# google/balloon-learning-environment

Measured on AMD Instinct MI355X. Metric: env-steps/sec at 65 536 parallel envs; achieved HBM GB/s fraction of peak, higher is better.
Workload: dtype f32+f64

## Files before the change

balloon_learning_environment_amd/csrc/ble_physics.h:

```cpp
#pragma once
#include "ble_intrinsics.h"

#ifndef BLE_STEP_EVENT
#define BLE_STEP_EVENT(i) do {} while (0)
#endif
#ifndef BLE_STEP_TICK
#define BLE_STEP_TICK(i) do {} while (0)
#endif

namespace ble {

constexpr float kGravity = 9.80665f;
constexpr double kGasConstantD = 8.3144621;
constexpr double kAirMolarMassD = 0.028964922481160;
constexpr double kHeMolarMassD = 0.004002602;
constexpr double kAirSpecificGasD = kGasConstantD / kAirMolarMassD;
constexpr float kAirMolarOverR = (float)(kAirMolarMassD / kGasConstantD);
constexpr float kGasConstant = (float)kGasConstantD;
constexpr double kPiD = 3.14159265358979323846;
constexpr float kPi = (float)kPiD;
constexpr float kDegToRad = (float)(kPiD / 180.0);
constexpr float kRadToDeg = (float)(180.0 / kPiD);

constexpr float kVolumeBase = 1804.0f;
// ... 75 lines not shown
  return d_fma(d_fma(-q0, b, x), rb, q0);
}
BLE_FN double d_rcp(double x) {
  double r = d_rcp_seed(x);
  return d_fma(d_fma(-x, r, 1.0), r, r);
}
BLE_FN double d_rsqrt(double x) {
  double y = d_rsq_seed(x);
  return y * d_fma(-0.5 * x * y, y, 1.5);
}
BLE_FN double d_sqrt_rs(double x) { return x * d_rsqrt(x); }
BLE_FN double d_sqrt_fast(double x) {
  double y = d_rsqrt(x);
  double sq = x * y;
  return d_fma(0.5 * y, d_fma(-sq, sq, x), sq);
}
constexpr double kThermalMu = 1.458e-6 / (0.028964922481160 / 8.3144621);
constexpr double kRayleighScale = 9.80665 * (1.0 / kThermalMu) * (1.0 / kThermalMu) * (6.0 / 3.14159265358979323846);
constexpr double kRayleighT = -3.25e-4 * kRayleighScale, kRayleighT0 = 0.804 * kRayleighScale;
constexpr double kEmitRho = 1.0 / (1.0 - 0.0291), kEmitC1 = 0.000232, kEmitC0 = 0.04587 - 0.000232 * 210.0;
constexpr double kEmitA = 0.000000056704 * (-kEmitRho * kEmitC1 * kEmitC1);
constexpr double kEmitB = 0.000000056704 * (2.0 * kEmitC1 - 2.0 * kEmitRho * kEmitC1 * kEmitC0);
constexpr double kEmitC = 0.000000056704 * (2.0 * kEmitC0 - kEmitRho * kEmitC0 * kEmitC0);
constexpr double kCondTenth = 0.1 * (0.0241 * 0.006415624181362592) / (2.0 * 0.62035049089940009);
struct StrideK {
  double ra_t0, five, eleven, emit_b, emit_c;
  double dry_mass;
  double lg5, lg4, lg3, ex4, ex3;
  double acs_x0, forty;
  double t110, cond_tenth;
  double m_over_r, ten;
  double lg6, ex5;
  double lift, v0;
};
BLE_FN StrideK stride_k_literal(double dry_mass = VehicleDefault::dry_mass, double lift = VehicleDefault::lift, double v0 = VehicleDefault::v0) {
  StrideK k;
  k.ra_t0 = kRayleighT0; k.five = 5.0; k.eleven = 11.0; k.emit_b = kEmitB; k.emit_c = kEmitC;
  k.dry_mass = dry_mass;
  k.lg5 = 0.2; k.lg4 = -0.25; k.lg3 = 1.0 / 3.0; k.ex4 = 1.0 / 24.0; k.ex3 = 1.0 / 6.0;
  k.acs_x0 = 0.05; k.forty = 40.0;
  k.t110 = 110.4; k.cond_tenth = kCondTenth;
  k.m_over_r = kAirMolarMassD / kGasConstantD; k.ten = 10.0;
  k.lg6 = -1.0 / 6.0; k.ex5 = 1.0 / 120.0;
  k.lift = lift; k.v0 = v0;
  return k;
}
BLE_FN StrideK stride_k_vreg(double dry_mass = VehicleDefault::dry_mass, double lift = VehicleDefault::lift, double v0 = VehicleDefault::v0) {
  StrideK k = stride_k_literal(dry_mass, lift, v0);
  k.ra_t0 = d_vreg(k.ra_t0); k.five = d_vreg(k.five); k.eleven = d_vreg(k.eleven); k.emit_b = d_vreg(k.emit_b); k.emit_c = d_vreg(k.emit_c);
  k.dry_mass = d_vreg(k.dry_mass);
  k.lg5 = d_vreg(k.lg5); k.lg4 = d_vreg(k.lg4); k.lg3 = d_vreg(k.lg3); k.ex4 = d_vreg(k.ex4); k.ex3 = d_vreg(k.ex3);
  k.acs_x0 = d_vreg(k.acs_x0); k.forty = d_vreg(k.forty);
  k.t110 = d_vreg(k.t110); k.cond_tenth = d_vreg(k.cond_tenth);
  k.m_over_r = d_vreg(k.m_over_r); k.ten = d_vreg(k.ten);
  k.lg6 = d_vreg(k.lg6); k.ex5 = d_vreg(k.ex5);
  k.lift = d_vreg(k.lift); k.v0 = d_vreg(k.v0);
  return k;
}
BLE_FN double d_log_fast(double x) {
  double m = d_frexp_mant(x);
  int e = d_frexp_exp(x);
  if (m < 0.70710678118654752) { m *= 2.0; e -= 1; }
  double sq = (m - 1.0) * d_rcp(m + 1.0);
  double z = sq * sq;
  double pl = 1.0 / 23.0;
  pl = d_fma(pl, z, 1.0 / 21.0); pl = d_fma(pl, z, 1.0 / 19.0); pl = d_fma(pl, z, 1.0 / 17.0);
  pl = d_fma(pl, z, 1.0 / 15.0); pl = d_fma(pl, z, 1.0 / 13.0); pl = d_fma(pl, z, 1.0 / 11.0);
  pl = d_fma(pl, z, 1.0 / 9.0); pl = d_fma(pl, z, 1.0 / 7.0); pl = d_fma(pl, z, 0.2);
  pl = d_fma(pl, z, 1.0 / 3.0);
  double lm = d_fma(2.0 * sq * z, pl, 2.0 * sq);
  double de = (double)e;
  return d_fma(de, 6.93147180369123816490e-01, d_fma(de, 1.90821492927058770002e-10, lm));
}
BLE_FN double d_exp_fast(double t) {
  double kq = d_rint(t * 1.44269504088896338700e+00);
  double r = d_fma(kq, -6.93147180369123816490e-01, t);
  r = d_fma(kq, -1.90821492927058770002e-10, r);
  double pe = 1.0 / 6227020800.0;
  pe = d_fma(pe, r, 1.0 / 479001600.0); pe = d_fma(pe, r, 1.0 / 39916800.0); pe = d_fma(pe, r, 1.0 / 3628800.0);
  pe = d_fma(pe, r, 1.0 / 362880.0); pe = d_fma(pe, r, 1.0 / 40320.0); pe = d_fma(pe, r, 1.0 / 5040.0);
  pe = d_fma(pe, r, 1.0 / 720.0); pe = d_fma(pe, r, 1.0 / 120.0); pe = d_fma(pe, r, 1.0 / 24.0);
  pe = d_fma(pe, r, 1.0 / 6.0); pe = d_fma(pe, r, 0.5); pe = d_fma(pe, r, 1.0); pe = d_fma(pe, r, 1.0);
  return d_ldexp(pe, (int)kq);
}
BLE_FN double d_pow_fast(double x, double y) { return d_exp_fast(y * d_log_fast(x)); }

constexpr float kLog2e = 1.4426950408889634f;
constexpr float kLn2 = 0.6931471805599453f;
BLE_FN float f_exp(float x) { return f_exp2(x * kLog2e); }
// ... 271 lines not shown
  double r = c0;
  r = j < 0 ? m1 : r;
  r = j > 0 ? p1 : r;
  return r;
}
BLE_FN double atm_height_rel_boundary_f64(double q, double pb, double r_pb, double tb, double lapse) {
  const double x = (q - pb) * r_pb;
  const double lg = x * d_fma(x, d_fma(x, d_fma(x, -0.25, 1.0 / 3.0), -0.5), 1.0);
  if (lapse == 0.0) return (-kAirSpecificGasD / 9.80665) * tb * lg;
  const double y = (-kAirSpecificGasD / 9.80665) * lapse * lg;
  const double em1 = y * d_fma(y, d_fma(y, d_fma(y, 1.0 / 24.0, 1.0 / 6.0), 0.5), 1.0);
  return (tb * em1) * d_rcp(lapse);
}
BLE_FN double atm_inv_delta_height_f64(const AtmWindow& w, int j, double lapse, double kl, double cur_hi, double cur_lo,
                                       double p, double rp, double d, double t_p, const StrideK& K = stride_k_literal()) {
  const double x = d * rp;
  const double lg = x * d_fma(x, d_fma(x, K.lg3, -0.5), 1.0);
  const bool iso = lapse == 0.0;
  const double y = kl * lg;
  const double em1 = y * d_fma(y, d_fma(y, K.ex3, 0.5), 1.0);
  double inv = lapse * d_rcp(t_p * em1);
  if (__builtin_expect(wave_any(iso), 0)) if (iso) inv = d_rcp(t_p * ((-kAirSpecificGasD / 9.80665) * lg));
  const double q = p + d;
  const bool below = q > cur_hi;
  const bool above = !(q > cur_lo);
  if (__builtin_expect(wave_any(below || above), 0)) if (below || above) {
    BLE_STEP_EVENT(2);
    const bool at_pb = (j == 0) ? below : (j < 0);
    const double pb = at_pb ? w.pb : w.pt, r_pb = at_pb ? w.r_pb : w.r_pt, tb = at_pb ? w.tb : w.tt;
    const double lapse_q = pick3(below ? j - 1 : j + 1, w.lapse_m1, w.lapse_0, w.lapse_p1);
    const double dh = atm_height_rel_boundary_f64(q, pb, r_pb, tb, lapse_q) -
                      atm_height_rel_boundary_f64(p, pb, r_pb, tb, lapse);
    inv = d_rcp(dh);
  }
  return inv;
}

BLE_FN int atm_window_layer(const AtmWindow& w, double p) { return p > w.pb ? -1 : (p > w.pt ? 0 : 1); }
BLE_FN AtmLayer atm_layer_f32(const AtmWindow& w, int j) {
  const float inf = __builtin_huge_valf();
  AtmLayer l;
  const float pb = (float)w.pb, pt = (float)w.pt, tb = (float)w.tb, tt = (float)w.tt;
  l.p_base = j < 0 ? inf : (j == 0 ? pb : pt);
  l.t_base = j == 0 ? tb : tt;
  l.p_top = j < 0 ? pb : (j == 0 ? pt : -inf);
  l.t_top = j < 0 ? tb : tt;
  const float lm1 = (float)w.lapse_m1, l0 = (float)w.lapse_0, lp1 = (float)w.lapse_p1;
  l.lapse = j < 0 ? lm1 : (j == 0 ? l0 : lp1);
  l.lapse_below = j <= 0 ? lm1 : l0;
  l.lapse_above = j < 0 ? l0 : lp1;
  l.h_base = (float)w.hb; l.k = -kROverG * l.lapse; l.index = w.i0 + j;
  return l;
}

BLE_FN int altitude_safety(int action, double altitude_m, uint8_t* fsm) {
  const double min_alt = 50000.0 * 0.3048, buffer = 500.0 * 0.3048, hyst = 500.0 * 0.3048;
  int s = *fsm;
  if (altitude_m < min_alt) s = 2;
  else if (altitude_m < min_alt + buffer) s = 1;
  else if (altitude_m < min_alt + buffer + hyst) s = (s == 2 || s == 1) ? 1 : 0;
  else s = 0;
  *fsm = (uint8_t)s;
  if (s == 2) return kUp;
  if (s == 1 && action == kDown) return kStay;
  return action;
}
// ... 450 lines not shown
  return f_fma(c35x4, sh33, c65x2 * sh27);
}
BLE_FN float solar_power_from_factor(float panel_factor, float attenuation) { return 210.0f * attenuation * panel_factor; }
BLE_FN float solar_power(const SunState& sun, float attenuation) {
  return solar_power_from_factor(solar_panel_factor(sun), attenuation);
}

constexpr float kSolarAbsorptivityTotal =
    0.01435f * (1.0f + (1.0f - 0.01435f - 0.0291f) / (1.0f - 0.0291f));
BLE_FN double d_inv_root4(double a, double five = 5.0) {
  const double y = (double)f_sqrt(f_rsqrt((float)a));
  const double y2 = y * y;
  return y * d_fma(-a * y2, y2, five) * 0.25;
}
BLE_FN double d_inv_root10(double a, double eleven = 11.0, double scale = 0.1) {
  const double y = (double)f_exp2(-0.1f * f_log2((float)a));
  const double y2 = y * y, y4 = y2 * y2, y5 = y4 * y;
  return y * d_fma(-a * y5, y5, eleven) * scale;
}
constexpr double kStefanBoltzmannD = 0.000000056704;
BLE_FN double total_absorptivity_d(double a) { return a * d_fma(-a, 1.0 / (1.0 - 0.0291), 2.0); }
constexpr double kAbsTLo = 0x1.891a7b9611a78p+3;
constexpr double kAbsTHi = 0x1.05f0e58469ee5p+13;
BLE_FN bool absorptivity_out_of_range(double t_k) { return t_k < kAbsTLo || t_k > kAbsTHi; }
constexpr float kAbsIrLo = 0x1.52847cp-10f;
constexpr float kAbsIrHi = 0x1.0af2d6p+28f;
BLE_FN bool earth_ir_out_of_range(double ir) { return ir < (double)kAbsIrLo || ir > (double)kAbsIrHi; }
BLE_FN double earth_heat_per_area_f64(double upwelling_ir, uint32_t* flags) {
  const double t_bb = d_sqrt(d_sqrt(upwelling_ir * (1.0 / kStefanBoltzmannD)));
  const double f = total_absorptivity_d(d_fma(0.000232, t_bb - 210.0, 0.04587));
  *flags |= earth_ir_out_of_range(upwelling_ir) ? kFlagAbsorptivity : 0u;
  return upwelling_ir * 0.4605 * f;
}
template <bool kExactTwelfthRoot = false>
BLE_FN double thermal_increment_f64(double vol, double yc, double t_int, double t_amb, double p, double q_solar_area,
                                    double q_earth_area, const StrideK& K = stride_k_literal(), double thermal_scale = VehicleDefault::thermal_scale) {
  constexpr double kR2 = 0.38483473658887897;
  constexpr double kR1 = 0.62035049089940009;
  const double v23 = vol * yc;
  const double t2 = t_int * t_int;
  const double q_emit = (t2 * t2) * d_fma(d_fma(kEmitA, t_int, K.emit_b), t_int, K.emit_c);
  const double rt = d_rcp(t_amb), rt2 = rt * rt, rt3 = rt2 * rt;
  const double pw = p * (t_amb + K.t110);
  const double dt = t_amb - t_int;
  double ra = (d_fma(kRayleighT, t_amb, K.ra_t0) * (pw * pw)) * ((vol * (rt3 * rt3)) * __builtin_fabs(dt));
  ra = d_max(ra, 1e-30);
  const double y4 = d_inv_root4(ra, K.five);
  const double ra14 = (ra * y4) * (y4 * y4);
  const double tw_arg = d_fma(2.69e-8, ra, 1.0);
  double tw = (double)f_pow((float)tw_arg, 1.0f / 12.0f);
  if (kExactTwelfthRoot) {
    const double y2 = tw * tw, y4r = y2 * y2, y8 = y4r * y4r;
    tw = d_fma(-tw * (1.0 / 12.0), d_fma(y8 * y4r, d_rcp(tw_arg), -1.0), tw);
  }
  const double nusselt = d_fma(0.457, ra14, 2.0 + tw);
  const double q_conv = ((nusselt * (t_amb * d_inv_root10(t_amb, K.eleven, K.cond_tenth))) * yc) * dt;
  const double q = (q_solar_area + q_earth_area) + (q_conv - q_emit);
  return (q * v23) * thermal_scale;
}

BLE_FN void superpressure_volume(float mols_air, float t_int, float p, float* volume, float* sp) {
  float vu = (kMolsLiftGas + mols_air) * kGasConstant * t_int * f_rcp(p);
  if (vu <= kVolumeBase) { *volume = vu; *sp = 0.0f; return; }
  float b = -(kVolumeBase - kVolumeDvDp * p);
  float c4 = 4.0f * kVolumeDvDp * vu * p;
  float v = 0.5f * (f_sqrt(f_fma(b, b, c4)) - b);
  *volume = v;
  *sp = p * (vu - v) * f_rcp(v);
}

BLE_FN void superpressure_volume_f64(double mols_air, double t_int, double p, double rp, double* volume, double* sp,
                                     const StrideK& K = stride_k_literal(), double dvdp = VehicleDefault::dvdp,
                                     double four_dvdp = VehicleDefault::four_dvdp, double inv_dvdp = VehicleDefault::inv_dvdp) {
  const double w = ((K.lift + mols_air) * kGasConstantD) * t_int;
  double vu = w * rp;
  double b = -(K.v0 - dvdp * p);
  double c4 = four_dvdp * w;
  double v = 0.5 * (d_sqrt_rs(d_fma(b, b, c4)) - b);
  bool slack = vu <= K.v0;
  *volume = slack ? vu : v;
  *sp = slack ? 0.0 : (v - K.v0) * inv_dvdp;
}

struct AcsEfficiencyTable { float v[4 * 13]; };
constexpr AcsEfficiencyTable kAcsEfficiencyValues = {{
    0.4f, 0.4f, 0.3f, 0.2f, 0.2f, 0.0f, 0.0f, 0.0f, 0.0f, 0.0f, 0.0f, 0.0f, 0.0f,
    0.4f, 0.3f, 0.3f, 0.30f, 0.25f, 0.23f, 0.20f, 0.15f, 0.12f, 0.10f, 0.0f, 0.0f, 0.0f,
    0.0f, 0.3f, 0.25f, 0.25f, 0.25f, 0.20f, 0.20f, 0.20f, 0.2f, 0.15f, 0.13f, 0.12f, 0.11f,
    0.0f, 0.23f, 0.23f, 0.23f, 0.23f, 0.23f, 0.20f, 0.20f, 0.20f, 0.18f, 0.16f, 0.15f, 0.13f}};
BLE_CONST_TABLE AcsEfficiencyTable kAcsEfficiencyTable = kAcsEfficiencyValues;
#define kAcsEfficiency (kAcsEfficiencyTable.v)
// ... 88 lines not shown
```

balloon_learning_environment_amd/csrc/ble_step_core.h:

```cpp
#pragma once
#include "ble_physics.h"

namespace ble {

struct StateDev {
  float *x, *y, *pressure, *ambient_temperature, *internal_temperature, *envelope_volume, *superpressure, *mols_air, *battery_charge;
  float *acs_power, *acs_mass_flow, *solar_charging, *power_load;
  const float *center_lat_deg, *center_lng_deg, *upwelling_infrared, *alpha;
  const int64_t* start_unix;
  int32_t *time_elapsed_s, *sunrise_h_rel, *sunset_rel;
  uint8_t *status, *last_command, *alt_fsm, *env_fsm, *power_paused;
  double* episode_cache;
};
struct EnvRegs {
  float x, y, p, t_amb, t_int, vol, sp, n_air, batt;
  float acs_power, mdot, charge, load;
  int32_t t_elapsed, sunrise_h, sunset;
  uint8_t status, alt_fsm, env_fsm, paused;
};
struct EnvConst {
  float lat0_deg, lng0_deg, ir, alpha;
  int64_t start_unix;
};
struct EnvHoisted {
// ... 40 lines not shown
}
BLE_FN EnvHoisted hoisted_from_cache(const EpisodeCacheRow& r, const EnvConst& c) {
  EnvHoisted h;
  atm_base_linear((double)c.alpha, &h.atm);
  h.atm.p1 = r.v[0]; h.atm.p2 = r.v[1];
  h.sin_lat0 = r.v[2]; h.cos_lat0 = r.v[3]; h.q_earth = r.v[4];
  uint64_t g2;
  __builtin_memcpy(&g2, &r.v[6], 8);
  h.flags = (uint32_t)(g2 & 0x7fffffffull);
  return h;
}


BLE_FN double inv_cbrt_volume(double vol) {
  double yc = (double)f_exp2((-1.0f / 3.0f) * f_log2((float)vol));
  return yc * d_fma(-vol * yc, yc * yc, 4.0) * (1.0 / 3.0);
}
BLE_FN double d_min_raw(double a, double b) {
#if defined(__HIP_DEVICE_COMPILE__)
  double r; asm("v_min_f64 %0, %1, %2" : "=v"(r) : "v"(a), "v"(b)); return r;
#else
  return d_min(a, b);
#endif
}
BLE_FN double d_max_raw(double a, double b) {
#if defined(__HIP_DEVICE_COMPILE__)
  double r; asm("v_max_f64 %0, %1, %2" : "=v"(r) : "v"(a), "v"(b)); return r;
#else
  return d_max(a, b);
#endif
}
struct LayerCursor {
  int lay;
  double lapse_cur;
  double kl_cur;
  double cur_hi, cur_lo;
};
BLE_FN double stride_pressure(const AtmWindow& win, const LayerCursor& lc, double p, double rp, double vol, double n_air,
                              double t_amb, double t_at_p, double yc, const StrideK& K, double drag_arg = VehicleDefault::drag_arg) {
  const double mass = d_fma(kAirMolarMassD, n_air, K.dry_mass);
  const double num = d_fma(p * vol, K.m_over_r, -mass * t_amb);
  const double dir = __builtin_copysign(1.0, num);
  const double arg = drag_arg * __builtin_fabs(num) * rp * (yc * yc);
  const double dh_dt = d_sqrt_rs(d_max(arg, 1e-30));
  const double inv_dh = atm_inv_delta_height_f64(win, lc.lay, lc.lapse_cur, lc.kl_cur, lc.cur_hi, lc.cur_lo, p, rp, dir, t_at_p, K);
  return d_fma(inv_dh * dh_dt, K.ten, p);
}
BLE_FN double stride_internal_temperature(double vol, double yc, double t_int, double t_amb, double p, float flux, float att,
                                          double q_earth, const StrideK& K, double thermal_scale = VehicleDefault::thermal_scale) {
  return t_int + thermal_increment_f64(vol, yc, t_int, t_amb, p, (double)((flux * att) * (0.25f * kSolarAbsorptivityTotal)), q_earth, K, thermal_scale);
}
BLE_FN void stride_acs(const double* acs_poly, int eff, double sp, double p, double rp, double t_int, float* acs_w, double* mdot_d,
                       const StrideK& K, double valve_k = VehicleDefault::valve_k) {
  const double a2 = d_max((2.0 * (kAirMolarMassD / kGasConstantD)) * (sp * (sp + p)), 1e-30);
  const double mdot_up = (valve_k * a2) * d_rsqrt(a2 * t_int);
  const double prm1 = d_max(sp * rp, 0.0);
  double w_down, mdot_down;
  acs_down_poly(acs_poly, prm1, &w_down, &mdot_down, K);
  *acs_w = eff == kDown ? (float)w_down : 0.0f;
  *mdot_d = eff == kUp ? mdot_up : (eff == kDown ? mdot_down : 0.0);
}
BLE_FN double stride_mols_air(double n_air, double mdot_d) {
  return d_max(d_fma(mdot_d, 10.0 / kAirMolarMassD, n_air), 0.0);
}
BLE_FN void stride_power_from_factor(bool is_day, float panel_factor, float att, float acs_w, float* charge, float* load, float* batt,
                                     float day_load = VehicleDefault::day_load, float night_load = VehicleDefault::night_load,
                                     float capacity = VehicleDefault::capacity) {
  *charge = is_day ? solar_power_from_factor(panel_factor, att) : 0.0f;
  *load = (is_day ? day_load : night_load) + acs_w;
  *batt = f_clamp(f_fma(*charge - *load, kStride / 3600.0f, *batt), 0.0f, capacity);
}
BLE_FN void stride_power(const SunState& sun, float att, float acs_w, float* charge, float* load, float* batt,
                         float day_load = VehicleDefault::day_load, float night_load = VehicleDefault::night_load,
                         float capacity = VehicleDefault::capacity) {
  stride_power_from_factor(sun.day, solar_panel_factor(sun), att, acs_w, charge, load, batt, day_load, night_load, capacity);
}
BLE_FN double stride_ambient_advance(const AtmWindow& win, LayerCursor& lc, double p, double rp, double t_at_p, double p_new,
                                     const StrideK& K) {
  const double kInf = (double)__builtin_huge_valf();
  double anchor_p = p, anchor_rp = rp, anchor_t = t_at_p;
  const bool crossed = p_new > lc.cur_hi || !(p_new > lc.cur_lo);
  if (__builtin_expect(wave_any(crossed), 0)) if (crossed) {
    BLE_STEP_EVENT(1);
    const int lay_new = atm_window_layer(win, p_new);
    const bool low_pair = (lc.lay + lay_new) < 0;
    anchor_p = low_pair ? win.pb : win.pt;
    anchor_rp = low_pair ? win.r_pb : win.r_pt;
    anchor_t = low_pair ? win.tb : win.tt;
    lc.lay = lay_new;
    lc.lapse_cur = pick3(lay_new, win.lapse_m1, win.lapse_0, win.lapse_p1);
    lc.kl_cur = (-kAirSpecificGasD / 9.80665) * lc.lapse_cur;
    lc.cur_hi = lay_new < 0 ? kInf : (lay_new == 0 ? win.pb : win.pt);
    lc.cur_lo = lay_new < 0 ? win.pb : (lay_new == 0 ? win.pt : -kInf);
  }
  return atm_temperature_advance(anchor_t, anchor_p, anchor_rp, p_new, lc.kl_cur, K);
}

struct SolarNodes {
  double sb0, cb0, sb1, cb1, sb2, cb2;
  double sd0, cd0, hsd, hcd;
};
BLE_FN SolarNodes solar_nodes_time(const Ephemeris& e0, int64_t t0, float lng0_deg, float step_s) {
  SolarNodes n;
  double sod;
  if (__builtin_expect(t0 >= 0 && t0 < 4294967296LL, 1)) sod = (double)((uint32_t)t0 % 86400u);
  else { int64_t m = t0 % 86400; sod = (double)(m < 0 ? m + 86400 : m); }
  const double b0 = sod * (1.0 / 240.0) + 0.25 * e0.eot_min + (double)lng0_deg;
  const double half_db = 0.5 * ((double)step_s * (1.0 / 240.0) + 0.25 * (double)(e0.eot_min_rate * step_s));
  double sb0, cb0;
  sincos_f64(b0 * (kPiD / 180.0), &sb0, &cb0);
  const double hr = half_db * (kPiD / 180.0), h2 = hr * hr;
  const double sh = hr * d_fma(h2, d_fma(h2, d_fma(h2, -1.0 / 5040.0, 1.0 / 120.0), -1.0 / 6.0), 1.0);
  const double ch = d_fma(h2, d_fma(h2, d_fma(h2, -1.0 / 720.0, 1.0 / 24.0), -0.5), 1.0);
  const double sb1 = sb0 * ch + cb0 * sh, cb1 = cb0 * ch - sb0 * sh;
  const double sb2 = sb1 * ch + cb1 * sh, cb2 = cb1 * ch - sb1 * sh;
  n.sb0 = sb0; n.cb0 = cb0; n.sb1 = sb1; n.cb1 = cb1; n.sb2 = sb2; n.cb2 = cb2;
  const double sd0 = (double)e0.sin_decl, cd0 = d_sqrt_fast(d_fma(-sd0, sd0, 1.0));
  const double hsd = 0.5 * (double)(e0.sin_decl_rate * step_s), hcd = -(sd0 * d_rcp(cd0)) * hsd;
  n.sd0 = sd0; n.cd0 = cd0; n.hsd = hsd; n.hcd = hcd;
  return n;
}
template <int j>
BLE_FN double solar_node(const SolarNodes& n, double sl0, double cl0, float x_m, float y_m, float u, float v, int substeps) {
  const double x0 = (double)x_m, y0 = (double)y_m;
  const double dx = (double)u * (5.0 * (double)substeps), dy = (double)v * (5.0 * (double)substeps);
  if (j == 0) return sun_one_minus_sin_f64(sl0, cl0, x0, y0, n.sb0, n.cb0, n.sd0, n.cd0);
// ... 44 lines not shown
    if (!excess) {
      const float scale = f_clamp((acs_power - 100.0f) * (1.0f / 200.0f), 0.0f, 1.0f);
      r *= f_fma(-0.3f, scale, 0.95f);
    }
  }
  return r;
}
template <typename SunFn>
BLE_FN float step_reward(int action, float x, float y, float p, float batt, float acs_power, SunFn sun_end,
                         float day_load = VehicleDefault::day_load, double capacity_wh = VehicleDefault::capacity_d) {
  return step_reward_from_power(action, x, y, batt, acs_power, [&]() {
    const SunState sun = sun_end();
    return solar_power(sun, solar_attenuation(sun.sin_el, p, sun.day));
  }, day_load, capacity_wh);
}

constexpr int kTermSaveRows = 14, kTermSaveStride = 64;
constexpr int kTermAbsBit = 1 << 16;
struct NoHelper { static constexpr bool kOn = false; };
struct SunRecord { float diff, panel_factor, flux; uint32_t bits; };
template <class V = VehicleDefault, class H = NoHelper>
BLE_FN int agent_step(EnvRegs& s, const EnvConst& c, const EnvHoisted& hc, int action, const WindCorners& corners, const WindQuery& wq,
                      float noise_u, float noise_v, int substeps, const double* acs_poly, const StrideK& K, float* term_save,
                      float* reward, uint32_t* flags, const V& veh = V(), H* helper = nullptr) {
  BLE_STEP_TICK(0);
  float u, v;
  if constexpr (H::kOn) {
    wind_blend_corners(corners, wq, &u, &v);
    u += noise_u; v += noise_v;
    helper->publish(s.x, s.y, u, v, s.t_elapsed);
  }
  const float p0_in = s.p;
  double p = (double)s.p;
  const AtmWindow win = atm_window_from(hc.atm, (double)c.alpha, p, flags);
  double altitude, t_at_p;
  atm_at_pressure_f64(win, (double)c.alpha, p, &altitude, &t_at_p);
  LayerCursor lc;
  lc.lay = 0; lc.lapse_cur = win.lapse_0; lc.kl_cur = (-kAirSpecificGasD / 9.80665) * win.lapse_0; lc.cur_hi = win.pb; lc.cur_lo = win.pt;

  int eff = action;
  if (veh.power_layer)
    eff = power_safety(action, s.t_elapsed, s.batt, &s.sunrise_h, &s.sunset, &s.paused, veh.night_load_d, veh.capacity_d);
  eff = envelope_safety(eff, s.sp, &s.env_fsm, veh.max_sp);
  eff = altitude_safety(eff, altitude, &s.alt_fsm);
  BLE_STEP_TICK(1);

  const int64_t t0 = c.start_unix + (int64_t)s.t_elapsed;
  const Ephemeris e0 = ephemeris(t0);
  const float step_s = (float)(10 * substeps);
  const float fl0 = e0.flux, dfl = e0.flux_rate * 10.0f;
  BLE_STEP_TICK(2);
  if constexpr (!H::kOn) {
    wind_blend_corners(corners, wq, &u, &v);
    u += noise_u; v += noise_v;
  }
  BLE_STEP_TICK(3);
  const SolarNodes nodes = solar_nodes_time(e0, t0, c.lng0_deg, step_s);
  const SunQuadratic sq = solar_nodes_site(nodes, hc.sin_lat0, hc.cos_lat0, s.x, s.y, u, v, substeps);
  BLE_STEP_TICK(4);
  const float x_start = s.x, y_start = s.y;
  const int32_t t_start = s.t_elapsed;
  auto sun_at = [&](int kk) -> SunState {
    return sun_at_stride(kk, sq, c, u, v, x_start, y_start, t_start);
  };
  const double q_earth = hc.q_earth;
  *flags |= hc.flags;

  double t_amb = (double)s.t_amb, t_int = (double)s.t_int, n_air = (double)s.n_air, vol = (double)s.vol,
         sp = (double)s.sp;
  double t_int_lo = t_int, t_int_hi = t_int;
  float x = s.x, y = s.y, batt = s.batt;
  float acs_w = s.acs_power, charge = s.charge, load = s.load;
  double mdot_d = (double)s.mdot;
  int status = kOk;

  float* const term_word = term_save + (kTermSaveRows - 1) * kTermSaveStride;
  *term_word = 0.0f;
  auto stride = [&](const int k) __attribute__((always_inline)) {
    const float pf = (float)p;
    const double rp = d_rcp(p);
    t_int_lo = d_min_raw(t_int_lo, t_int); t_int_hi = d_max_raw(t_int_hi, t_int);
    SunState sun;
    SunRecord rec;
    float flux;
    if constexpr (!H::kOn) {
      const float fk = (float)k;
      sun = sun_at(k);
      flux = f_fma(fk, dfl, fl0);
    } else {
      rec = helper->record(k);
      flux = rec.flux;
    }

    const double yc = inv_cbrt_volume(vol);
    const double p_new = stride_pressure(win, lc, p, rp, vol, n_air, t_amb, t_at_p, yc, K, veh.drag_arg);

    float att;
    if constexpr (!H::kOn) att = solar_attenuation(sun.sin_el, pf, sun.day);
    else att = solar_attenuation_from_diff(rec.diff, pf, (rec.bits & 1u) != 0);
    const double t_int_new = stride_internal_temperature(vol, yc, t_int, t_amb, p, flux, att, q_earth, K, veh.thermal_scale);

    double vol_new, sp_new;
    superpressure_volume_f64(n_air, t_int, p, rp, &vol_new, &sp_new, K, veh.dvdp, veh.four_dvdp, veh.inv_dvdp);
    bool terminal = !(sp_new <= veh.max_sp) || sp_new <= 0.0;

    stride_acs(acs_poly, eff, sp, p, rp, t_int, &acs_w, &mdot_d, K, veh.valve_k);
    const double n_air_new = stride_mols_air(n_air, mdot_d);

    if constexpr (!H::kOn) stride_power(sun, att, acs_w, &charge, &load, &batt, veh.day_load, veh.night_load, veh.capacity);
    else stride_power_from_factor((rec.bits & 1u) != 0, rec.panel_factor, att, acs_w, &charge, &load, &batt, veh.day_load, veh.night_load, veh.capacity);
    terminal = terminal || batt <= 0.0f;

    x = f_fma(u, kStride, x);
    y = f_fma(v, kStride, y);
    t_amb = t_at_p;
    t_at_p = stride_ambient_advance(win, lc, p, rp, t_at_p, p_new, K);
    p = p_new; t_int = t_int_new; vol = vol_new; sp = sp_new; n_air = n_air_new;
    if (__builtin_expect(wave_any(terminal), 0)) if (terminal && __builtin_bit_cast(int, *term_word) == 0) {
      int st = kOk;
      if (!(sp <= veh.max_sp)) st = kBurst;
      if (sp <= 0.0) st = kZeroPressure;
      if (batt <= 0.0f) st = kOutOfPower;
      const float parked[kTermSaveRows - 1] = {x, y, (float)p, (float)t_amb, (float)t_int, (float)vol, (float)sp, (float)n_air, batt,
                                               acs_w, (float)mdot_d, charge, load};
#pragma unroll
      for (int j = 0; j < kTermSaveRows - 1; ++j) term_save[j * kTermSaveStride] = parked[j];
      const int strides = i_opaque(k + 1);
      const int abs_bad = absorptivity_out_of_range(t_int_lo) || absorptivity_out_of_range(t_int_hi) ? kTermAbsBit : 0;
      *term_word = __builtin_bit_cast(float, st | (strides << 8) | abs_bad);
      if constexpr (H::kOn) helper->park_reward_record(k + 1);
    }
  };
  int ks = 0;
#pragma unroll 1
  for (; ks + 1 < substeps; ks += 2) { stride(ks); stride(ks + 1); }
  if (ks < substeps) stride(ks);
  BLE_STEP_TICK(5);
  s.x = x; s.y = y; s.p = (float)p; s.t_amb = (float)t_amb; s.t_int = (float)t_int; s.vol = (float)vol;
  s.sp = (float)sp; s.n_air = (float)n_air; s.batt = batt;
  s.acs_power = acs_w; s.mdot = (float)mdot_d; s.charge = charge; s.load = load;
  int k = substeps;
  const int word = __builtin_bit_cast(int, *term_word);
  const bool done = word != 0;
  SunRecord rec_end;
  if constexpr (H::kOn) rec_end = helper->record_end(substeps);
  bool abs_bad = absorptivity_out_of_range(t_int_lo) || absorptivity_out_of_range(t_int_hi);
  if (__builtin_expect(wave_any(done), 0)) if (done) {
    s.x = term_save[0]; s.y = term_save[kTermSaveStride]; s.p = term_save[2 * kTermSaveStride]; s.t_amb = term_save[3 * kTermSaveStride];
    s.t_int = term_save[4 * kTermSaveStride]; s.vol = term_save[5 * kTermSaveStride]; s.sp = term_save[6 * kTermSaveStride];
// ... 24 lines not shown
```

balloon_learning_environment_amd/csrc/ble_step_split.h:

```cpp
#pragma once
#include "ble_noise.h"
#include "ble_step_core.h"

#ifdef BLE_SPLIT_TIMING
#define BLE_SPLIT_T_DECL long long t_acc[6] = {0, 0, 0, 0, 0, 0}; long long t_last = (long long)__builtin_readcyclecounter()
#define BLE_SPLIT_T(sec) do { const long long t_now = (long long)__builtin_readcyclecounter(); t_acc[sec] += t_now - t_last; t_last = t_now; } while (0)
#define BLE_SPLIT_T_FLUSH(dbg, role) do { if ((dbg) != nullptr && lane == 0) { for (int q = 0; q < 6; ++q) atomicAdd((dbg) + (role) * 8 + q, (unsigned long long)t_acc[q]); atomicAdd((dbg) + (role) * 8 + 7, 1ull); } } while (0)
#else
#define BLE_SPLIT_T_DECL do {} while (0)
#define BLE_SPLIT_T(sec) do {} while (0)
#define BLE_SPLIT_T_FLUSH(dbg, role) do {} while (0)
#endif

namespace ble {

constexpr int kSplitWaves = 4;
constexpr int kSplitLanes = 64;

struct SplitShared {
  double acs_poly[kAcsPolyDoubles];
  double p[2][kSplitLanes], t_amb[2][kSplitLanes];
  float x[2][kSplitLanes], y[2][kSplitLanes];
  double t_int[2][kSplitLanes];
  float sin_el[2][kSplitLanes], panel[2][kSplitLanes]; uint32_t day[2][kSplitLanes];
// ... 77 lines not shown
      noise_draws_fetch(a.gen.seed, (uint64_t)i, (uint64_t)(i + a.gen.env_offset), a.gen.episode ? a.gen.episode[i] : 0u, a.gen.harmonic_cache, n,
                        &shn.draws[0][lane], kSplitLanes);
  }
  __syncthreads();
  const bool was_live = live;
  int last_act = 0;
  EnvHoisted hc;
  if (in_range && st.episode_cache != nullptr && episode_cache_hit(cached, c)) {
    hc = hoisted_from_cache(cached, c);
  } else {
    hc = hoist_constants(c);
    if (r0 && live && st.episode_cache != nullptr) episode_cache_store(st.episode_cache, n, i, c, hc);
  }
  int xk = 0;
  BLE_SPLIT_T_DECL;

#pragma unroll 1
  for (int step = 0; step < a.n_steps; ++step) {
    const int64_t o = (int64_t)step * n + i;
    int act = kStay;
    if (in_range) act = a.action[o];
    if (live) last_act = act;

    double p = (double)s.p, t_amb = (double)s.t_amb, t_int = (double)s.t_int, n_air = (double)s.n_air, vol = (double)s.vol,
           sp = (double)s.sp;
    float x = s.x, y = s.y, batt = s.batt;
    float acs_w = 0.0f, mdot = 0.0f, charge = 0.0f, load = 0.0f;
    float u = 0.0f, v = 0.0f;
    const float p0_in = s.p, x_start = s.x, y_start = s.y;
    const int32_t t_start = s.t_elapsed;
    const int64_t t0 = c.start_unix + (int64_t)s.t_elapsed;
    const float step_s = (float)(10 * substeps);
    uint32_t step_flags = 0;
    AtmWindow win = {}; LayerCursor lc = {}; double t_at_p = 0.0;
    float fl0 = 0.0f, dfl = 0.0f; Ephemeris e0 = {};
    SunQuadratic sq = {}; double node_f0 = 0.0;
    float sun_sin = 0.0f, sun_panel = 0.0f; bool sun_day = false;
    uint32_t map_pow_env = 0; int eff = kStay;

    if (r1) {
      e0 = ephemeris(t0);
      fl0 = e0.flux; dfl = e0.flux_rate * 10.0f;
      sh.eot_min[lane] = e0.eot_min; sh.eph[0][lane] = e0.eot_min_rate; sh.eph[1][lane] = e0.sin_decl; sh.eph[2][lane] = e0.sin_decl_rate;
      step_flags |= hc.flags;
    }
    if (r3) {
      int32_t sr0 = s.sunrise_h, ss0 = s.sunset, sr1 = s.sunrise_h, ss1 = s.sunset, sr2 = s.sunrise_h, ss2 = s.sunset;
      uint8_t pa0 = s.paused, pa1 = s.paused, pa2 = s.paused, f0 = s.env_fsm, f1 = s.env_fsm, f2 = s.env_fsm;
      const int q0 = envelope_safety(power_safety(kDown, s.t_elapsed, s.batt, &sr0, &ss0, &pa0), s.sp, &f0);
      const int q1 = envelope_safety(power_safety(kStay, s.t_elapsed, s.batt, &sr1, &ss1, &pa1), s.sp, &f1);
      const int q2 = envelope_safety(power_safety(kUp, s.t_elapsed, s.batt, &sr2, &ss2, &pa2), s.sp, &f2);
      if (live) { s.sunrise_h = sr0; s.sunset = ss0; s.paused = pa0; s.env_fsm = f0; }
      map_pow_env = action_map(q0, q1, q2);
    }
    if constexpr (kNoise) {
      if (in_range) {
        float x_km, y_km, t_h;
        noise_coords(s.x, s.y, s.t_elapsed, &x_km, &y_km, &t_h);
#pragma unroll 1
        for (int k = wave; k < 10; k += kSplitWaves)
          shn.nz[k][lane] = noise_harmonic_value(k / 5, k % 5, harmonic_draw_from_rows(&shn.draws[0][lane], kSplitLanes, k), x_km, y_km, s.p, t_h,
                                                 shn.grad_lut);
      }
      __syncthreads();
    }
    if (r2) {
      const WindQuery wq = wind_query(s.x, s.y, s.p, s.t_elapsed);
      WindCorners corners;
      wind_gather(a.wind_grid + (in_range ? i : 0) * a.grid_env_stride, wq, &corners);
      float nu = 0.0f, nv = 0.0f;
      if constexpr (kNoise) {
        if (in_range) wind_noise_from_values(&shn.nz[0][lane], kSplitLanes, &nu, &nv);
      } else {
        if (a.noise_uv && in_range) { nu = a.noise_uv[2 * i]; nv = a.noise_uv[2 * i + 1]; }
      }
      wind_blend_corners(corners, wq, &u, &v);
      u += nu; v += nv;
      sh.u[lane] = u; sh.v[lane] = v;
    }
    BLE_SPLIT_T(0);
    __syncthreads();
    BLE_SPLIT_T(1);
    if (!r2) { u = sh.u[lane]; v = sh.v[lane]; }
    if (!r1) { e0.eot_min = sh.eot_min[lane]; e0.eot_min_rate = sh.eph[0][lane]; e0.sin_decl = sh.eph[1][lane]; e0.sin_decl_rate = sh.eph[2][lane]; }
    if (r0) {
      win = atm_window_from(hc.atm, (double)c.alpha, p, &step_flags);
      lc.lay = 0; lc.lapse_cur = win.lapse_0; lc.kl_cur = (-kAirSpecificGasD / 9.80665) * win.lapse_0; lc.cur_hi = win.pb; lc.cur_lo = win.pt;
      double altitude;
      atm_at_pressure_f64(win, (double)c.alpha, p, &altitude, &t_at_p);
      uint8_t f0 = s.alt_fsm, f1 = s.alt_fsm, f2 = s.alt_fsm;
      const int q0 = altitude_safety(kDown, altitude, &f0), q1 = altitude_safety(kStay, altitude, &f1),
                q2 = altitude_safety(kUp, altitude, &f2);
      if (live) s.alt_fsm = f0;
      sh.map_alt[lane] = action_map(q0, q1, q2);
    }
    if (r1 || r2 || r3) {
      const SolarNodes nd = solar_nodes_time(e0, t0, c.lng0_deg, step_s);
      if (r1) sh.node_f[0][lane] = solar_node<1>(nd, hc.sin_lat0, hc.cos_lat0, s.x, s.y, u, v, substeps);
      if (r3) sh.node_f[1][lane] = solar_node<2>(nd, hc.sin_lat0, hc.cos_lat0, s.x, s.y, u, v, substeps);
      if (r2) {
        node_f0 = solar_node<0>(nd, hc.sin_lat0, hc.cos_lat0, s.x, s.y, u, v, substeps);
        sq.c0 = (float)node_f0; sq.c1 = 0.0f; sq.c2 = 0.0f; sq.thr = sun_thresholds(node_f0, substeps);
        const SunState sun0 = sun_at_stride(0, sq, c, u, v, x_start, y_start, t_start);
        sun_sin = sun0.sin_el; sun_panel = solar_panel_factor(sun0); sun_day = sun0.day;
        sh.sin_el0[lane] = sun_sin; sh.panel0[lane] = sun_panel; sh.day0[lane] = sun_day ? 1u : 0u;
      }
    }
    BLE_SPLIT_T(0);
    __syncthreads();
    BLE_SPLIT_T(1);
    if (r2) sq = solar_node_coefs(node_f0, sh.node_f[0][lane], sh.node_f[1][lane], substeps);
    if (r1 || r3) { sun_sin = sh.sin_el0[lane]; sun_panel = sh.panel0[lane]; sun_day = sh.day0[lane] != 0u; }
    if (r3) eff = action_apply_any(sh.map_alt[lane], map_pow_env, act);
    if (live) flags |= step_flags;

    bool active = live;
    bool abs_bad = false;
    int k_done = 0, last_rd = 0, status = kOk;
    const StrideK K = stride_k_vreg();
#pragma unroll 1
    for (int k = 0; k < substeps; ++k) {
      if (__ballot(active) == 0ull) break;
      const int wr = (xk + 1) & 1;
      const bool publish = active || !live;
      double p_n = p, t_amb_n = t_amb, t_at_p_n = t_at_p, t_int_n = t_int, vol_n = vol, sp_n = sp, n_air_n = n_air;
      float x_n = x, y_n = y, batt_n = batt, sun_sin_n = sun_sin, sun_panel_n = sun_panel; bool sun_day_n = sun_day;
      const double rp = d_rcp(p);
      if (r0) {
        const double yc = inv_cbrt_volume(vol);
        p_n = stride_pressure(win, lc, p, rp, vol, n_air, t_amb, t_at_p, yc, K);
        x_n = f_fma(u, kStride, x); y_n = f_fma(v, kStride, y);
        t_amb_n = t_at_p;
        t_at_p_n = stride_ambient_advance(win, lc, p, rp, t_at_p, p_n, K);
        if (publish) { sh.p[wr][lane] = p_n; sh.t_amb[wr][lane] = t_amb_n; sh.x[wr][lane] = x_n; sh.y[wr][lane] = y_n; }
      }
      if (r1) {
        abs_bad = abs_bad || (active && absorptivity_out_of_range(t_int));
        const float flux = f_fma((float)k, dfl, fl0);
        const double yc = inv_cbrt_volume(vol);
        const float att = solar_attenuation(sun_sin, (float)p, sun_day);
        t_int_n = stride_internal_temperature(vol, yc, t_int, t_amb, p, flux, att, hc.q_earth, K);
        if (publish) sh.t_int[wr][lane] = t_int_n;
      }
      if (r2) {
        const SunState sn = sun_at_stride(k + 1, sq, c, u, v, x_start, y_start, t_start);
        sun_sin_n = sn.sin_el; sun_panel_n = solar_panel_factor(sn); sun_day_n = sn.day;
        if (publish) { sh.sin_el[wr][lane] = sun_sin_n; sh.panel[wr][lane] = sun_panel_n; sh.day[wr][lane] = sun_day_n ? 1u : 0u; }
        superpressure_volume_f64(n_air, t_int, p, rp, &vol_n, &sp_n, K);
        const uint32_t code = sp_n <= 0.0 ? (uint32_t)kZeroPressure : (!(sp_n <= 2380.0) ? (uint32_t)kBurst : 0u);
        if (publish) { sh.vol[wr][lane] = vol_n; sh.sp[wr][lane] = sp_n; sh.code_sp[wr][lane] = code; }
      }
      if (r3) {
        const float att = solar_attenuation(sun_sin, (float)p, sun_day);
        double mdot_d;
        stride_acs(sh.acs_poly, eff, sp, p, rp, t_int, &acs_w, &mdot_d, K);
        mdot = (float)mdot_d;
        n_air_n = stride_mols_air(n_air, mdot_d);
        stride_power_from_factor(sun_day, sun_panel, att, acs_w, &charge, &load, &batt_n);
        if (publish) {
          sh.n_air[wr][lane] = n_air_n; sh.batt[wr][lane] = batt_n; sh.acs_w[wr][lane] = acs_w; sh.mdot[wr][lane] = mdot;
          sh.charge[wr][lane] = charge; sh.load[wr][lane] = load;
          sh.code_batt[wr][lane] = batt_n <= 0.0f ? (uint32_t)kOutOfPower : 0u;
        }
      }
      BLE_SPLIT_T(2);
      __syncthreads();
      BLE_SPLIT_T(3);
      ++xk;
      const int rd = xk & 1;
      if (r0) { p = p_n; t_amb = t_amb_n; t_at_p = t_at_p_n; x = x_n; y = y_n; } else { p = sh.p[rd][lane]; }
      if (r1) { t_int = t_int_n; t_amb = sh.t_amb[rd][lane]; } else if (r2 || r3) t_int = sh.t_int[rd][lane];
      if (r2) { vol = vol_n; sp = sp_n; sun_sin = sun_sin_n; sun_panel = sun_panel_n; sun_day = sun_day_n; }
      else { if (r0 || r1) vol = sh.vol[rd][lane]; if (r3) sp = sh.sp[rd][lane]; }
      if (r3) { n_air = n_air_n; batt = batt_n; } else if (r0 || r2) n_air = sh.n_air[rd][lane];
      if (r1 || r3) { sun_sin = sh.sin_el[rd][lane]; sun_day = sh.day[rd][lane] != 0u; if (r3) sun_panel = sh.panel[rd][lane]; }
      const uint32_t cb = sh.code_batt[rd][lane], cs = sh.code_sp[rd][lane];
      const int code = (int)(cb != 0u ? cb : cs);
      k_done = active ? k + 1 : k_done; last_rd = active ? rd : last_rd; status = active ? code : status;
      active = active && code == kOk;
      BLE_SPLIT_T(4);
    }

    if (live) {
      const int rd = last_rd;
      s.p = (float)sh.p[rd][lane]; s.t_amb = (float)sh.t_amb[rd][lane]; s.t_int = (float)sh.t_int[rd][lane];
      s.vol = (float)sh.vol[rd][lane]; s.sp = (float)sh.sp[rd][lane]; s.n_air = (float)sh.n_air[rd][lane];
      s.batt = sh.batt[rd][lane]; s.x = sh.x[rd][lane]; s.y = sh.y[rd][lane];
      s.t_elapsed += 10 * k_done;
      s.status = (uint8_t)status;
      if (r1) flags |= abs_bad ? kFlagAbsorptivity : 0u;
      if (r0) {
        s.acs_power = sh.acs_w[rd][lane];
        flags |= (s.p > 101325.0f || s.p < 0.0f || p0_in > 101325.0f || p0_in < 0.0f) ? kFlagSolarRange : 0u;
        SunState sun_end = {};
        sun_end.sin_el = sh.sin_el[rd][lane]; sun_end.day = sh.day[rd][lane] != 0u;
        const float panel_end = sh.panel[rd][lane];
        float r = reward_distance(s.x, s.y);
        if (act == kDown) {
          const float pw = solar_power_from_factor(panel_end, solar_attenuation(sun_end.sin_el, s.p, sun_end.day));
          const bool excess = (pw > kDayLoad) && battery_above_99_percent(s.batt);
          if (!excess) {
            const float scale = f_clamp((s.acs_power - 100.0f) * (1.0f / 200.0f), 0.0f, 1.0f);
            r *= f_fma(-0.3f, scale, 0.95f);
// ... 43 lines not shown
```

Measured before the change: 4.809 billion.

## Replace log/exp inverse height with series in reciprocal pressure and share reciprocal temperatures

Replaces the per-stride inverse delta-height computation (log and expm1 series plus a reciprocal) with a truncated series in 1/p, scaled by 1/T at pressure and folding the -R/g factor into a new constant. The reciprocal of ambient temperature is carried across strides so the thermal increment can reuse it instead of recomputing it. The atmosphere base is built from a linear base with hoisted p1/p2. This removes double-precision transcendental work from the hot loop. In exchange it adds a carried register and relies on the series being accurate enough for unit pressure steps.

Result: no change. 4.832 billion (median of 6 runs) (+0.5%).

```diff
diff --git a/balloon_learning_environment_amd/csrc/ble_physics.h b/balloon_learning_environment_amd/csrc/ble_physics.h
--- a/balloon_learning_environment_amd/csrc/ble_physics.h
+++ b/balloon_learning_environment_amd/csrc/ble_physics.h
@@ -131,6 +131,7 @@
   double m_over_r, ten;
   double lg6, ex5;
   double lift, v0;
+  double ten_g_r;
 };
 BLE_FN StrideK stride_k_literal(double dry_mass = VehicleDefault::dry_mass, double lift = VehicleDefault::lift, double v0 = VehicleDefault::v0) {
   StrideK k;
@@ -142,6 +143,7 @@
   k.m_over_r = kAirMolarMassD / kGasConstantD; k.ten = 10.0;
   k.lg6 = -1.0 / 6.0; k.ex5 = 1.0 / 120.0;
   k.lift = lift; k.v0 = v0;
+  k.ten_g_r = 10.0 * (-9.80665 / kAirSpecificGasD);
   return k;
 }
 BLE_FN StrideK stride_k_vreg(double dry_mass = VehicleDefault::dry_mass, double lift = VehicleDefault::lift, double v0 = VehicleDefault::v0) {
@@ -154,6 +156,7 @@
   k.m_over_r = d_vreg(k.m_over_r); k.ten = d_vreg(k.ten);
   k.lg6 = d_vreg(k.lg6); k.ex5 = d_vreg(k.ex5);
   k.lift = d_vreg(k.lift); k.v0 = d_vreg(k.v0);
+  k.ten_g_r = d_vreg(k.ten_g_r);
   return k;
 }
 BLE_FN double d_log_fast(double x) {
@@ -491,6 +494,28 @@
     const double dh = atm_height_rel_boundary_f64(q, pb, r_pb, tb, lapse_q) -
                       atm_height_rel_boundary_f64(p, pb, r_pb, tb, lapse);
     inv = d_rcp(dh);
+  }
+  return inv;
+}
+BLE_FN double atm_inv_dh_c2(double kl) { return d_fma(kl, kl * (1.0 / 12.0), -1.0 / 12.0); }
+BLE_FN double atm_inv_delta_height_rg(const AtmWindow& w, int j, double kl, double c2, double cur_hi, double cur_lo,
+                                      double p, double rp, double num, double r_p) {
+  const double x = __builtin_copysign(rp, num);
+  const double c1 = d_fma(kl, -0.5, 0.5);
+  const double s = d_fma(x, d_fma(c2 * x, d_fma(x, -0.5, 1.0), c1), 1.0);
+  double inv = (__builtin_copysign(p, num) * r_p) * s;
+  const double d = __builtin_copysign(1.0, num);
+  const double q = p + d;
+  const bool below = q > cur_hi;
+  const bool above = !(q > cur_lo);
+  if (__builtin_expect(wave_any(below || above), 0)) if (below || above) {
+    BLE_STEP_EVENT(2);
+    const bool at_pb = (j == 0) ? below : (j < 0);
+    const double pb = at_pb ? w.pb : w.pt, r_pb = at_pb ? w.r_pb : w.r_pt, tb = at_pb ? w.tb : w.tt;
+    const double lapse_q = pick3(below ? j - 1 : j + 1, w.lapse_m1, w.lapse_0, w.lapse_p1);
+    const double dh = atm_height_rel_boundary_f64(q, pb, r_pb, tb, lapse_q) -
+                      atm_height_rel_boundary_f64(p, pb, r_pb, tb, pick3(j, w.lapse_m1, w.lapse_0, w.lapse_p1));
+    inv = (-kAirSpecificGasD / 9.80665) * d_rcp(dh);
   }
   return inv;
 }
@@ -1007,15 +1032,15 @@
   *flags |= earth_ir_out_of_range(upwelling_ir) ? kFlagAbsorptivity : 0u;
   return upwelling_ir * 0.4605 * f;
 }
-template <bool kExactTwelfthRoot = false>
-BLE_FN double thermal_increment_f64(double vol, double yc, double t_int, double t_amb, double p, double q_solar_area,
-                                    double q_earth_area, const StrideK& K = stride_k_literal(), double thermal_scale = VehicleDefault::thermal_scale) {
+template <bool kExactTwelfthRoot = false, bool kGivenRt = true>
+BLE_FN double thermal_increment_core(double vol, double yc, double t_int, double t_amb, double rt_given, double p, double q_solar_area,
+                                     double q_earth_area, const StrideK& K = stride_k_literal(), double thermal_scale = VehicleDefault::thermal_scale) {
   constexpr double kR2 = 0.38483473658887897;
   constexpr double kR1 = 0.62035049089940009;
   const double v23 = vol * yc;
   const double t2 = t_int * t_int;
   const double q_emit = (t2 * t2) * d_fma(d_fma(kEmitA, t_int, K.emit_b), t_int, K.emit_c);
-  const double rt = d_rcp(t_amb), rt2 = rt * rt, rt3 = rt2 * rt;
+  const double rt = kGivenRt ? rt_given : d_rcp(t_amb), rt2 = rt * rt, rt3 = rt2 * rt;
   const double pw = p * (t_amb + K.t110);
   const double dt = t_amb - t_int;
   double ra = (d_fma(kRayleighT, t_amb, K.ra_t0) * (pw * pw)) * ((vol * (rt3 * rt3)) * __builtin_fabs(dt));
@@ -1032,6 +1057,11 @@
   const double q_conv = ((nusselt * (t_amb * d_inv_root10(t_amb, K.eleven, K.cond_tenth))) * yc) * dt;
   const double q = (q_solar_area + q_earth_area) + (q_conv - q_emit);
   return (q * v23) * thermal_scale;
+}
+template <bool kExactTwelfthRoot = false>
+BLE_FN double thermal_increment_f64(double vol, double yc, double t_int, double t_amb, double p, double q_solar_area,
+                                    double q_earth_area, const StrideK& K = stride_k_literal(), double thermal_scale = VehicleDefault::thermal_scale) {
+  return thermal_increment_core<kExactTwelfthRoot, false>(vol, yc, t_int, t_amb, 0.0, p, q_solar_area, q_earth_area, K, thermal_scale);
 }
 
 BLE_FN void superpressure_volume(float mols_air, float t_int, float p, float* volume, float* sp) {
diff --git a/balloon_learning_environment_amd/csrc/ble_step_core.h b/balloon_learning_environment_amd/csrc/ble_step_core.h
--- a/balloon_learning_environment_amd/csrc/ble_step_core.h
+++ b/balloon_learning_environment_amd/csrc/ble_step_core.h
@@ -96,23 +96,31 @@
 }
 struct LayerCursor {
   int lay;
-  double lapse_cur;
   double kl_cur;
+  double c2;
   double cur_hi, cur_lo;
 };
+BLE_FN void layer_cursor_set(LayerCursor& lc, const AtmWindow& win, int lay) {
+  const double kInf = (double)__builtin_huge_valf();
+  lc.lay = lay;
+  lc.kl_cur = (-kAirSpecificGasD / 9.80665) * pick3(lay, win.lapse_m1, win.lapse_0, win.lapse_p1);
+  lc.c2 = atm_inv_dh_c2(lc.kl_cur);
+  lc.cur_hi = lay < 0 ? kInf : (lay == 0 ? win.pb : win.pt);
+  lc.cur_lo = lay < 0 ? win.pb : (lay == 0 ? win.pt : -kInf);
+}
 BLE_FN double stride_pressure(const AtmWindow& win, const LayerCursor& lc, double p, double rp, double vol, double n_air,
-                              double t_amb, double t_at_p, double yc, const StrideK& K, double drag_arg = VehicleDefault::drag_arg) {
+                              double t_amb, double r_at_p, double yc, const StrideK& K, double drag_arg = VehicleDefault::drag_arg) {
   const double mass = d_fma(kAirMolarMassD, n_air, K.dry_mass);
   const double num = d_fma(p * vol, K.m_over_r, -mass * t_amb);
-  const double dir = __builtin_copysign(1.0, num);
   const double arg = drag_arg * __builtin_fabs(num) * rp * (yc * yc);
   const double dh_dt = d_sqrt_rs(d_max(arg, 1e-30));
-  const double inv_dh = atm_inv_delta_height_f64(win, lc.lay, lc.lapse_cur, lc.kl_cur, lc.cur_hi, lc.cur_lo, p, rp, dir, t_at_p, K);
-  return d_fma(inv_dh * dh_dt, K.ten, p);
-}
-BLE_FN double stride_internal_temperature(double vol, double yc, double t_int, double t_amb, double p, float flux, float att,
+  const double inv_dh_rg = atm_inv_delta_height_rg(win, lc.lay, lc.kl_cur, lc.c2, lc.cur_hi, lc.cur_lo, p, rp, num, r_at_p);
+  return d_fma(inv_dh_rg * dh_dt, K.ten_g_r, p);
+}
+BLE_FN double stride_internal_temperature(double vol, double yc, double t_int, double t_amb, double r_amb, double p, float flux, float att,
                                           double q_earth, const StrideK& K, double thermal_scale = VehicleDefault::thermal_scale) {
-  return t_int + thermal_increment_f64(vol, yc, t_int, t_amb, p, (double)((flux * att) * (0.25f * kSolarAbsorptivityTotal)), q_earth, K, thermal_scale);
+  return t_int + thermal_increment_core(vol, yc, t_int, t_amb, r_amb, p, (double)((flux * att) * (0.25f * kSolarAbsorptivityTotal)), q_earth, K,
+                                        thermal_scale);
 }
 BLE_FN void stride_acs(const double* acs_poly, int eff, double sp, double p, double rp, double t_int, float* acs_w, double* mdot_d,
                        const StrideK& K, double valve_k = VehicleDefault::valve_k) {
@@ -141,7 +149,6 @@
 }
 BLE_FN double stride_ambient_advance(const AtmWindow& win, LayerCursor& lc, double p, double rp, double t_at_p, double p_new,
                                      const StrideK& K) {
-  const double kInf = (double)__builtin_huge_valf();
   double anchor_p = p, anchor_rp = rp, anchor_t = t_at_p;
   const bool crossed = p_new > lc.cur_hi || !(p_new > lc.cur_lo);
   if (__builtin_expect(wave_any(crossed), 0)) if (crossed) {
@@ -151,11 +158,7 @@
     anchor_p = low_pair ? win.pb : win.pt;
     anchor_rp = low_pair ? win.r_pb : win.r_pt;
     anchor_t = low_pair ? win.tb : win.tt;
-    lc.lay = lay_new;
-    lc.lapse_cur = pick3(lay_new, win.lapse_m1, win.lapse_0, win.lapse_p1);
-    lc.kl_cur = (-kAirSpecificGasD / 9.80665) * lc.lapse_cur;
-    lc.cur_hi = lay_new < 0 ? kInf : (lay_new == 0 ? win.pb : win.pt);
-    lc.cur_lo = lay_new < 0 ? win.pb : (lay_new == 0 ? win.pt : -kInf);
+    layer_cursor_set(lc, win, lay_new);
   }
   return atm_temperature_advance(anchor_t, anchor_p, anchor_rp, p_new, lc.kl_cur, K);
 }
@@ -266,11 +269,14 @@
   }
   const float p0_in = s.p;
   double p = (double)s.p;
-  const AtmWindow win = atm_window_from(hc.atm, (double)c.alpha, p, flags);
+  AtmBase ab;
+  atm_base_linear(d_vreg((double)c.alpha), &ab);
+  ab.p1 = hc.atm.p1; ab.p2 = hc.atm.p2;
+  const AtmWindow win = atm_window_from(ab, (double)c.alpha, p, flags);
   double altitude, t_at_p;
   atm_at_pressure_f64(win, (double)c.alpha, p, &altitude, &t_at_p);
   LayerCursor lc;
-  lc.lay = 0; lc.lapse_cur = win.lapse_0; lc.kl_cur = (-kAirSpecificGasD / 9.80665) * win.lapse_0; lc.cur_hi = win.pb; lc.cur_lo = win.pt;
+  layer_cursor_set(lc, win, 0);
 
   int eff = action;
   if (veh.power_layer)
@@ -302,6 +308,7 @@
 
   double t_amb = (double)s.t_amb, t_int = (double)s.t_int, n_air = (double)s.n_air, vol = (double)s.vol,
          sp = (double)s.sp;
+  double r_amb = d_rcp(t_amb), r_at_p = d_rcp(t_at_p);
   double t_int_lo = t_int, t_int_hi = t_int;
   float x = s.x, y = s.y, batt = s.batt;
   float acs_w = s.acs_power, charge = s.charge, load = s.load;
@@ -327,12 +334,12 @@
     }
 
     const double yc = inv_cbrt_volume(vol);
-    const double p_new = stride_pressure(win, lc, p, rp, vol, n_air, t_amb, t_at_p, yc, K, veh.drag_arg);
+    const double p_new = stride_pressure(win, lc, p, rp, vol, n_air, t_amb, r_at_p, yc, K, veh.drag_arg);
 
     float att;
     if constexpr (!H::kOn) att = solar_attenuation(sun.sin_el, pf, sun.day);
     else att = solar_attenuation_from_diff(rec.diff, pf, (rec.bits & 1u) != 0);
-    const double t_int_new = stride_internal_temperature(vol, yc, t_int, t_amb, p, flux, att, q_earth, K, veh.thermal_scale);
+    const double t_int_new = stride_internal_temperature(vol, yc, t_int, t_amb, r_amb, p, flux, att, q_earth, K, veh.thermal_scale);
 
     double vol_new, sp_new;
     superpressure_volume_f64(n_air, t_int, p, rp, &vol_new, &sp_new, K, veh.dvdp, veh.four_dvdp, veh.inv_dvdp);
@@ -347,8 +354,9 @@
 
     x = f_fma(u, kStride, x);
     y = f_fma(v, kStride, y);
-    t_amb = t_at_p;
+    t_amb = t_at_p; r_amb = r_at_p;
     t_at_p = stride_ambient_advance(win, lc, p, rp, t_at_p, p_new, K);
+    r_at_p = d_rcp(t_at_p);
     p = p_new; t_int = t_int_new; vol = vol_new; sp = sp_new; n_air = n_air_new;
     if (__builtin_expect(wave_any(terminal), 0)) if (terminal && __builtin_bit_cast(int, *term_word) == 0) {
       int st = kOk;
diff --git a/balloon_learning_environment_amd/csrc/ble_step_split.h b/balloon_learning_environment_amd/csrc/ble_step_split.h
--- a/balloon_learning_environment_amd/csrc/ble_step_split.h
+++ b/balloon_learning_environment_amd/csrc/ble_step_split.h
@@ -133,7 +133,7 @@
     const int64_t t0 = c.start_unix + (int64_t)s.t_elapsed;
     const float step_s = (float)(10 * substeps);
     uint32_t step_flags = 0;
-    AtmWindow win = {}; LayerCursor lc = {}; double t_at_p = 0.0;
+    AtmWindow win = {}; LayerCursor lc = {}; double t_at_p = 0.0, r_at_p = 0.0;
     float fl0 = 0.0f, dfl = 0.0f; Ephemeris e0 = {};
     SunQuadratic sq = {}; double node_f0 = 0.0;
     float sun_sin = 0.0f, sun_panel = 0.0f; bool sun_day = false;
@@ -186,9 +186,10 @@
     if (!r1) { e0.eot_min = sh.eot_min[lane]; e0.eot_min_rate = sh.eph[0][lane]; e0.sin_decl = sh.eph[1][lane]; e0.sin_decl_rate = sh.eph[2][lane]; }
     if (r0) {
       win = atm_window_from(hc.atm, (double)c.alpha, p, &step_flags);
-      lc.lay = 0; lc.lapse_cur = win.lapse_0; lc.kl_cur = (-kAirSpecificGasD / 9.80665) * win.lapse_0; lc.cur_hi = win.pb; lc.cur_lo = win.pt;
+      layer_cursor_set(lc, win, 0);
       double altitude;
       atm_at_pressure_f64(win, (double)c.alpha, p, &altitude, &t_at_p);
+      r_at_p = d_rcp(t_at_p);
       uint8_t f0 = s.alt_fsm, f1 = s.alt_fsm, f2 = s.alt_fsm;
       const int q0 = altitude_safety(kDown, altitude, &f0), q1 = altitude_safety(kStay, altitude, &f1),
                 q2 = altitude_safety(kUp, altitude, &f2);
@@ -224,15 +225,16 @@
       if (__ballot(active) == 0ull) break;
       const int wr = (xk + 1) & 1;
       const bool publish = active || !live;
-      double p_n = p, t_amb_n = t_amb, t_at_p_n = t_at_p, t_int_n = t_int, vol_n = vol, sp_n = sp, n_air_n = n_air;
+      double p_n = p, t_amb_n = t_amb, t_at_p_n = t_at_p, r_at_p_n = r_at_p, t_int_n = t_int, vol_n = vol, sp_n = sp, n_air_n = n_air;
       float x_n = x, y_n = y, batt_n = batt, sun_sin_n = sun_sin, sun_panel_n = sun_panel; bool sun_day_n = sun_day;
       const double rp = d_rcp(p);
       if (r0) {
         const double yc = inv_cbrt_volume(vol);
-        p_n = stride_pressure(win, lc, p, rp, vol, n_air, t_amb, t_at_p, yc, K);
+        p_n = stride_pressure(win, lc, p, rp, vol, n_air, t_amb, r_at_p, yc, K);
         x_n = f_fma(u, kStride, x); y_n = f_fma(v, kStride, y);
         t_amb_n = t_at_p;
         t_at_p_n = stride_ambient_advance(win, lc, p, rp, t_at_p, p_n, K);
+        r_at_p_n = d_rcp(t_at_p_n);
         if (publish) { sh.p[wr][lane] = p_n; sh.t_amb[wr][lane] = t_amb_n; sh.x[wr][lane] = x_n; sh.y[wr][lane] = y_n; }
       }
       if (r1) {
@@ -240,7 +242,7 @@
         const float flux = f_fma((float)k, dfl, fl0);
         const double yc = inv_cbrt_volume(vol);
         const float att = solar_attenuation(sun_sin, (float)p, sun_day);
-        t_int_n = stride_internal_temperature(vol, yc, t_int, t_amb, p, flux, att, hc.q_earth, K);
+        t_int_n = stride_internal_temperature(vol, yc, t_int, t_amb, d_rcp(t_amb), p, flux, att, hc.q_earth, K);
         if (publish) sh.t_int[wr][lane] = t_int_n;
       }
       if (r2) {
@@ -269,7 +271,7 @@
       BLE_SPLIT_T(3);
       ++xk;
       const int rd = xk & 1;
-      if (r0) { p = p_n; t_amb = t_amb_n; t_at_p = t_at_p_n; x = x_n; y = y_n; } else { p = sh.p[rd][lane]; }
+      if (r0) { p = p_n; t_amb = t_amb_n; t_at_p = t_at_p_n; r_at_p = r_at_p_n; x = x_n; y = y_n; } else { p = sh.p[rd][lane]; }
       if (r1) { t_int = t_int_n; t_amb = sh.t_amb[rd][lane]; } else if (r2 || r3) t_int = sh.t_int[rd][lane];
       if (r2) { vol = vol_n; sp = sp_n; sun_sin = sun_sin_n; sun_panel = sun_panel_n; sun_day = sun_day_n; }
       else { if (r0 || r1) vol = sh.vol[rd][lane]; if (r3) sp = sh.sp[rd][lane]; }
```
